# yl4579/StyleTTS2

Hardware: AMD Instinct MI355X
Metric: audio-seconds/sec (RTF^-1) end-to-end, 10 s utterance batch (higher is better)
Workload: dtype f32 (convs/linears: f16 hi/lo split, 3 MFMA products, fp32 accumulate)

## Files before the change

### styletts2_amd/_build.py

```python
import os
import subprocess
import sys

HERE = os.path.dirname(os.path.abspath(__file__))
CSRC = os.path.join(HERE, "csrc")
INCLUDE = os.path.join(os.path.dirname(HERE), "include")
LIB_PATH = os.path.join(HERE, "libst2_hip.so")

SOURCES = ["st2_api.hip", "st2_conv1d.hip", "st2_conv1d_f16s.hip", "st2_conv1d_f16s_k0.hip", "st2_conv1d_f16s_k1.hip",
           "st2_conv1d_f16s_k2.hip", "st2_conv1d_f16s_w0.hip", "st2_conv1d_f16s_w1.hip", "st2_conv1d_f16s_w2.hip",
           "st2_conv1d_xs.hip", "st2_conv1d_xs_k0.hip", "st2_conv1d_xs_k1.hip",
           "st2_conv1d_xs_k2.hip", "st2_conv1d_xs_k3.hip", "st2_actsplit.hip", "st2_norm.hip", "st2_misc.hip", "st2_glue.hip", "st2_pack.hip", "st2_resample.hip", "st2_passage.hip", "st2_level.hip", "st2_limit.hip", "st2_rng.hip", "st2_fit.hip", "st2_ingest.hip", "st2_controls.hip", "st2_marks.hip", "st2_style.hip", "st2_engine.hip", "st2_source.hip", "st2_attention.hip", "st2_lstm.hip", "st2_lstm_coop.hip", "st2_probe.hip", "st2_probe_conv.hip"]
FLAGS = ["--offload-arch=gfx950", "-O3", "-std=c++17", "-ffp-contract=off", "-fPIC", "-Wall",
         "-Wno-unused-function", "-I" + INCLUDE, "-I" + CSRC]
EXTRA_FLAGS = {s: ["-fno-slp-vectorize"] for s in SOURCES if s.startswith("st2_conv1d_f16s_k")}
EXTRA_FLAGS.update({"st2_lstm.hip": ["-fno-slp-vectorize"], "st2_lstm_coop.hip": ["-fno-slp-vectorize"]})
EXTRA_FLAGS.update({"st2_resample.hip": ["-fno-slp-vectorize"], "st2_ingest.hip": ["-fno-slp-vectorize"]})
EXTRA_FLAGS.update({"st2_level.hip": ["-fno-slp-vectorize"]})
EXTRA_FLAGS.update({"st2_limit.hip": ["-fno-slp-vectorize"]})


def _hipcc():
    for c in (os.environ.get("HIPCC"), "/opt/rocm/bin/hipcc", "hipcc"):
        if c and (os.path.isabs(c) and os.path.exists(c) or not os.path.isabs(c)):
            return c
    raise RuntimeError("hipcc not found")


def _newer(src_list, target):
    if not os.path.exists(target):
        return True
    t = os.path.getmtime(target)
    return any((not os.path.exists(s)) or os.path.getmtime(s) > t for s in src_list)


def _depfile_inputs(depfile):
    try:
        text = open(depfile).read()
    except OSError:
        return None
    text = text.replace("\\\n", " ")
    if ":" not in text:
        return None
    deps = text.split(":", 1)[1].split()
    return [d for d in deps if not d.startswith("/opt/rocm") and not d.startswith("/usr/")] or None


def _stale(src, obj, flags):
    stamp = obj + ".flags"
    try:
        if open(stamp).read() != " ".join(flags):
            return True
    except OSError:
        return True
    deps = _depfile_inputs(obj[:-2] + ".d")
    return deps is None or _newer([src] + deps, obj)


def build_lib(force=False, verbose=True):
    hipcc = _hipcc()
    objdir = os.path.join(CSRC, "build")
    os.makedirs(objdir, exist_ok=True)
    objs = []
    procs = []
    for s in SOURCES:
        src = os.path.join(CSRC, s)
        obj = os.path.join(objdir, s.replace(".hip", ".o"))
        objs.append(obj)
        flags = FLAGS + EXTRA_FLAGS.get(s, [])
        if force or _stale(src, obj, flags):
            cmd = [hipcc] + flags + ["-MD", "-MF", obj[:-2] + ".d", "-c", src, "-o", obj]
            if verbose:
                print("[st2 build]", " ".join(cmd), flush=True)
            if os.path.exists(obj + ".flags"):
                os.remove(obj + ".flags")
            procs.append((s, obj, flags, subprocess.Popen(cmd)))
    for s, obj, flags, p in procs:
        if p.wait() != 0:
            raise RuntimeError("hipcc failed on %s" % s)
        with open(obj + ".flags", "w") as f:
            f.write(" ".join(flags))
    if force or procs or _newer(objs, LIB_PATH):
        cmd = [hipcc, "--offload-arch=gfx950", "-shared", "-fPIC", "-o", LIB_PATH] + objs
        if verbose:
            print("[st2 build]", " ".join(cmd), flush=True)
        subprocess.check_call(cmd)
        isa_gate(verbose)
    return LIB_PATH


def isa_gate(verbose=True):
    import importlib.util
    path = os.path.join(os.path.dirname(HERE), "tools", "check_isa.py")
    spec = importlib.util.spec_from_file_location("st2_check_isa", path)
    mod = importlib.util.module_from_spec(spec)
    spec.loader.exec_module(mod)
    ok, report = mod.check(LIB_PATH)
    if verbose or ok is False:
        print("[st2 build] " + report, flush=True)
    if ok is False:
        os.replace(LIB_PATH, LIB_PATH + ".rejected")
        raise RuntimeError("libst2_hip.so failed the ISA gate (tools/check_isa.py); kept as %s.rejected" % LIB_PATH)
    return ok


if __name__ == "__main__":
    build_lib(force="--force" in sys.argv)
    print(LIB_PATH)
```

### styletts2_amd/csrc/st2_misc.hip

```cpp
#include "st2_common.h"

namespace {

__global__ __launch_bounds__(256) void conv1d_direct_kernel(const float* __restrict__ x, int64_t x_bs, int x_cs,
                                                            const float* __restrict__ w,
                                                            const float* __restrict__ bias, float* __restrict__ y,
                                                            int64_t y_bs, int y_cs, int C_in, int L_in_max, int L_out,
                                                            int ks, int stride, int pad, const int32_t* __restrict__ x_len,
                                                            const int32_t* __restrict__ y_len) {
  const int l = blockIdx.x * 256 + threadIdx.x;
  const int co = blockIdx.y;
  const int b = blockIdx.z;
  if (l >= L_out) return;
  const int L_in = x_len ? min(x_len[b], L_in_max) : L_in_max;
  if (y_len && l >= y_len[b]) {
    y[(int64_t)b * y_bs + (int64_t)co * y_cs + l] = 0.f;
    return;
  }
  const float* xb = x + (int64_t)b * x_bs;
  const float* wc = w + (int64_t)co * C_in * ks;
  float acc = 0.f;
  const int base = l * stride - pad;
  for (int ci = 0; ci < C_in; ++ci) {
    const float* xr = xb + (int64_t)ci * x_cs;
    for (int t = 0; t < ks; ++t) {
      const int p = base + t;
      if (p >= 0 && p < L_in) acc = fmaf(wc[ci * ks + t], xr[p], acc);
    }
  }
  if (bias) acc += bias[co];
  y[(int64_t)b * y_bs + (int64_t)co * y_cs + l] = acc;
}

__global__ __launch_bounds__(256) void phase_split_kernel(const float* __restrict__ x, int64_t x_bs, int x_cs, int L_in,
                                                          float* __restrict__ xp, int64_t p_bs, int p_cs, int Lu,
                                                          int stride, int pad) {
  const int pp = blockIdx.x * 256 + threadIdx.x;
  const int ci = blockIdx.y;
  const int b = blockIdx.z;
  if (pp >= Lu * stride) return;
  const int u = pp / stride;
  const int r = pp - u * stride;
  const int p = pp - pad;
  const float v = (p >= 0 && p < L_in) ? x[(int64_t)b * x_bs + (int64_t)ci * x_cs + p] : 0.f;
  xp[(int64_t)b * p_bs + (int64_t)(ci * stride + r) * p_cs + u] = v;
}

constexpr int CVT_TILE = 1024;
template <int S>
__global__ __launch_bounds__(256) void convt_interleave_kernel(const float* __restrict__ ph, int64_t p_bs, int p_cs,
                                                               const float* __restrict__ bias,
                                                               const float* __restrict__ add, int64_t a_bs, int a_cs,
                                                               float* __restrict__ out, int64_t o_bs, int o_cs, int C,
                                                               int stride_rt, int pad, int L_raw_max, int reflect_left,
                                                               float* __restrict__ part, int part_nt, int Lq_max,
                                                               const int32_t* __restrict__ q_len,
                                                               const int32_t* __restrict__ out_len) {
  extern __shared__ float cvt_tile[];
  __shared__ float red[2][4];
  const int stride = S ? S : stride_rt;
  const int co = blockIdx.y;
  const int b = blockIdx.z;
  const int L_out = out_len ? min(out_len[b], L_raw_max + reflect_left) : L_raw_max + reflect_left;
  const int Lq = q_len ? min(q_len[b], Lq_max) : Lq_max;
  const int o0 = blockIdx.x * CVT_TILE;
  if (o0 >= L_out) return;
  const int nq = CVT_TILE / stride + 3;
  const int nqp = nq | 1;
  const int l_lo = max(o0 - reflect_left, 0);
  const int q_lo = (l_lo + pad) / stride;
  {
    const float* pb = ph + (int64_t)b * p_bs + (int64_t)co * p_cs;
    const int total = stride * nq;
    constexpr int SB = 8;
    for (int e0 = threadIdx.x; e0 < total; e0 += 256 * SB) {
      float t[SB];
#pragma unroll
      for (int u = 0; u < SB; ++u) {
        const int e = min(e0 + u * 256, total - 1);
        const int r = e / nq, i = e - r * nq;
        t[u] = pb[(int64_t)r * C * p_cs + max(min(q_lo + i, Lq - 1), 0)];
      }
#pragma unroll
      for (int u = 0; u < SB; ++u) {
        const int e = e0 + u * 256;
        if (e < total) {
          const int r = e / nq, i = e - r * nq;
          cvt_tile[r * nqp + i] = (q_lo + i) < Lq ? t[u] : 0.f;
        }
      }
    }
  }
  __syncthreads();
  const float bj = bias ? bias[co] : 0.f;
  const float* ab = add ? add + (int64_t)b * a_bs + (int64_t)co * a_cs : nullptr;
  float* ob = out + (int64_t)b * o_bs + (int64_t)co * o_cs;
  auto staged_at = [&](int o) __attribute__((always_inline)) -> float {
    int l = o;
    if (reflect_left) l = (o == 0) ? 1 : o - 1;
    const int lp = l + pad;
    const int q = lp / stride;
    const int r = lp - q * stride;
    return cvt_tile[r * nqp + (q - q_lo)] + bj;
  };
  float shift = staged_at(o0);
  if (ab) shift += ab[o0];
  float s1 = 0.f, s2 = 0.f;
  const int o = o0 + 4 * threadIdx.x;
  if (o < L_out) {
    typedef float f4 __attribute__((ext_vector_type(4)));
    const bool full = o + 3 < L_out;
    const bool vec = full && ((reinterpret_cast<uintptr_t>(ob + o) & 15) == 0) && (!ab || (reinterpret_cast<uintptr_t>(ab + o) & 15) == 0);
    float v[4];
#pragma unroll
    for (int e = 0; e < 4; ++e) v[e] = (full || o + e < L_out) ? staged_at(o + e) : 0.f;
    if (ab) {
      if (vec) {
        const f4 a4 = *reinterpret_cast<const f4*>(ab + o);
#pragma unroll
        for (int e = 0; e < 4; ++e) v[e] += a4[e];
      } else {
#pragma unroll
        for (int e = 0; e < 4; ++e)
          if (full || o + e < L_out) v[e] += ab[o + e];
      }
    }
    if (vec) {
      *reinterpret_cast<f4*>(ob + o) = f4{v[0], v[1], v[2], v[3]};
    } else {
#pragma unroll
      for (int e = 0; e < 4; ++e)
        if (full || o + e < L_out) ob[o + e] = v[e];
    }
#pragma unroll
    for (int e = 0; e < 4; ++e)
      if (full || o + e < L_out) {
        const float dv = v[e] - shift;
        s1 += dv;
        s2 += dv * dv;
      }
  }
  if (part) {
    s1 = st2_wave_sum(s1);
    s2 = st2_wave_sum(s2);
    const int lane = threadIdx.x & 63, wave = threadIdx.x >> 6;
    if (lane == 0) {
      red[0][wave] = s1;
      red[1][wave] = s2;
    }
    __syncthreads();
    if (threadIdx.x == 0) {
      const float t1 = ((red[0][0] + red[0][1]) + red[0][2]) + red[0][3];
      const float t2 = ((red[1][0] + red[1][1]) + red[1][2]) + red[1][3];
      const int64_t slot = ((int64_t)b * C + co) * part_nt + blockIdx.x;
      reinterpret_cast<float2*>(part)[slot] = make_float2(t1, t2);
      part[(int64_t)gridDim.z * C * part_nt * 2 + slot] = shift;
    }
  }
}

__global__ __launch_bounds__(256) void adain_leaky_pool_kernel(const float* __restrict__ x, int64_t x_bs, int x_cs,
                                                               const float* __restrict__ stats,
                                                               const float* __restrict__ gamma,
                                                               const float* __restrict__ beta, int64_t gb_bs,
                                                               float slope, const float* __restrict__ w,
                                                               const float* __restrict__ bias, float* __restrict__ y,
                                                               int64_t y_bs, int y_cs, int C, int L_max,
                                                               const int32_t* __restrict__ len) {
  const int lo = blockIdx.x * 256 + threadIdx.x;
  const int c = blockIdx.y;
  const int b = blockIdx.z;
  const int L = len ? min(len[b], L_max) : L_max;
  if (lo >= 2 * L) return;
  const float mean = stats[((int64_t)b * C + c) * 2 + 0];
  const float rstd = stats[((int64_t)b * C + c) * 2 + 1];
  const float g = 1.0f + gamma[(int64_t)b * gb_bs + c];
  const float be = beta[(int64_t)b * gb_bs + c];
  const float* xr = x + (int64_t)b * x_bs + (int64_t)c * x_cs;
  auto act = [&](int i) -> float {
    float u = (xr[i] - mean) * rstd;
    u = g * u + be;
    return u >= 0.f ? u : u * slope;
  };
  const int j = lo >> 1;
  float v;
  if ((lo & 1) == 0) {
    v = act(j) * w[c * 3 + 1];
  } else {
    v = act(j) * w[c * 3 + 2];
    if (j + 1 < L) v += act(j + 1) * w[c * 3 + 0];
  }
  if (bias) v += bias[c];
  y[(int64_t)b * y_bs + (int64_t)c * y_cs + lo] = v;
}

__global__ __launch_bounds__(256) void add_chanvec_kernel(const float* __restrict__ x, int64_t x_bs, int x_cs,
                                                          const float* __restrict__ v, int64_t v_bs,
                                                          float* __restrict__ y, int64_t y_bs, int y_cs, int C,
                                                          int N) {
  const int n = blockIdx.x * 256 + threadIdx.x;
  const int c = blockIdx.y;
  const int b = blockIdx.z;
  if (n >= N) return;
  y[(int64_t)b * y_bs + (int64_t)c * y_cs + n] =
      x[(int64_t)b * x_bs + (int64_t)c * x_cs + n] + v[(int64_t)b * v_bs + c];
}

__global__ __launch_bounds__(64) void mean_tokens_kernel(const float* __restrict__ x, int64_t x_bs, int x_cs,
                                                         float* __restrict__ m, int64_t m_bs, int C, int N,
                                                         const int* __restrict__ len) {
  const int c = blockIdx.x;
  const int b = blockIdx.y;
  const float* xr = x + (int64_t)b * x_bs + (int64_t)c * x_cs;
  const int n_b = len ? min(max(len[b], 1), N) : N;
  double s = 0.0;
  for (int n = threadIdx.x; n < n_b; n += 64) s += (double)xr[n];
  s = st2_wave_sum(s);
  if (threadIdx.x == 0) m[(int64_t)b * m_bs + c] = (float)(s / (double)n_b);
}

__global__ __launch_bounds__(256) void axpbypcz_kernel(const float* __restrict__ x, float a,
                                                       const float* __restrict__ y, float b,
                                                       const float* __restrict__ z, float c, float* __restrict__ out,
                                                       int64_t n) {
  const int64_t i = (int64_t)blockIdx.x * 256 + threadIdx.x;
  if (i >= n) return;
  float v = a * x[i];
  if (y) v += b * y[i];
  if (z) v += c * z[i];
  out[i] = v;
}

}

extern "C" int st2_conv1d_direct(const float* x, int64_t x_bs, int32_t x_cs, const float* w, const float* bias,
                                 float* y, int64_t y_bs, int32_t y_cs, int32_t B, int32_t C_in, int32_t C_out,
                                 int32_t L_in, int32_t L_out, int32_t ks, int32_t stride, int32_t pad,
                                 void* stream) {
  return st2_conv1d_direct_len(x, x_bs, x_cs, w, bias, y, y_bs, y_cs, B, C_in, C_out, L_in, L_out, ks, stride, pad, nullptr,
                               nullptr, stream);
}

extern "C" int st2_conv1d_direct_len(const float* x, int64_t x_bs, int32_t x_cs, const float* w, const float* bias,
                                     float* y, int64_t y_bs, int32_t y_cs, int32_t B, int32_t C_in, int32_t C_out,
                                     int32_t L_in, int32_t L_out, int32_t ks, int32_t stride, int32_t pad,
                                     const int32_t* x_len, const int32_t* y_len, void* stream) {
  ST2_REQUIRE(x && w && y && B > 0 && C_in > 0 && C_out > 0 && L_in > 0 && L_out > 0 && ks > 0 && stride > 0,
              "st2_conv1d_direct: bad arguments");
  ST2_REQUIRE(C_out <= 65535 && B <= 65535, "st2_conv1d_direct: grid too large");
  hipStream_t s = reinterpret_cast<hipStream_t>(stream);
  hipLaunchKernelGGL(conv1d_direct_kernel, dim3(st2_cdiv(L_out, 256), C_out, B), dim3(256), 0, s, x, x_bs, x_cs, w,
                     bias, y, y_bs, y_cs, C_in, L_in, L_out, ks, stride, pad, x_len, y_len);
  ST2_CHECK_LAUNCH("st2_conv1d_direct");
  return 0;
}

extern "C" int st2_phase_split(const float* x, int64_t x_bs, int32_t x_cs, int32_t B, int32_t C, int32_t L_in,
                               int32_t stride, int32_t pad, float* xp, int64_t p_bs, int32_t p_cs, int32_t Lu,
                               void* stream) {
  ST2_REQUIRE(x && xp && B > 0 && C > 0 && L_in > 0 && stride > 0 && pad >= 0 && Lu > 0,
              "st2_phase_split: bad arguments");
  ST2_REQUIRE(C <= 65535 && B <= 65535 && (int64_t)Lu * stride < (int64_t)1 << 31, "st2_phase_split: grid too large");
  hipStream_t s = reinterpret_cast<hipStream_t>(stream);
  hipLaunchKernelGGL(phase_split_kernel, dim3(st2_cdiv((int64_t)Lu * stride, 256), C, B), dim3(256), 0, s, x, x_bs,
                     x_cs, L_in, xp, p_bs, p_cs, Lu, stride, pad);
  ST2_CHECK_LAUNCH("st2_phase_split");
  return 0;
}

extern "C" int st2_convt_interleave(const float* phases, int64_t p_bs, int32_t p_cs, int32_t Lq, const float* bias,
                                    const float* add, int64_t a_bs, int32_t a_cs, float* out, int64_t o_bs,
                                    int32_t o_cs, int32_t B, int32_t C, int32_t stride, int32_t pad, int32_t L_raw,
                                    int32_t reflect_left, void* stream) {
  return st2_convt_interleave_stats(phases, p_bs, p_cs, Lq, bias, add, a_bs, a_cs, out, o_bs, o_cs, B, C, stride, pad,
                                    L_raw, reflect_left, nullptr, 0, stream);
}

extern "C" int st2_convt_interleave_stats(const float* phases, int64_t p_bs, int32_t p_cs, int32_t Lq,
                                          const float* bias, const float* add, int64_t a_bs, int32_t a_cs, float* out,
                                          int64_t o_bs, int32_t o_cs, int32_t B, int32_t C, int32_t stride, int32_t pad,
                                          int32_t L_raw, int32_t reflect_left, float* part, int32_t part_nt,
                                          void* stream) {
  return st2_convt_interleave_stats_len(phases, p_bs, p_cs, Lq, bias, add, a_bs, a_cs, out, o_bs, o_cs, B, C, stride, pad, L_raw,
                                        reflect_left, part, part_nt, nullptr, nullptr, stream);
}

extern "C" int st2_convt_interleave_stats_len(const float* phases, int64_t p_bs, int32_t p_cs, int32_t Lq,
                                              const float* bias, const float* add, int64_t a_bs, int32_t a_cs, float* out,
                                              int64_t o_bs, int32_t o_cs, int32_t B, int32_t C, int32_t stride, int32_t pad,
                                              int32_t L_raw, int32_t reflect_left, float* part, int32_t part_nt,
                                              const int32_t* q_len, const int32_t* out_len, void* stream) {
  ST2_REQUIRE(!q_len == !out_len, "st2_convt_interleave_stats_len: q_len and out_len go together");
  ST2_REQUIRE(phases && out && B > 0 && C > 0 && stride > 0 && L_raw > 0 && Lq > 0,
              "st2_convt_interleave: bad arguments");
  ST2_REQUIRE(reflect_left == 0 || (reflect_left == 1 && L_raw >= 2), "st2_convt_interleave: bad reflect_left");
  ST2_REQUIRE(stride <= 64, "st2_convt_interleave: stride %d too large", stride);
  const int L_out = L_raw + reflect_left;
  const int nt = st2_cdiv(L_out, CVT_TILE);
  if (part) ST2_REQUIRE(part_nt >= nt && (reinterpret_cast<uintptr_t>(part) & 7) == 0,
                        "st2_convt_interleave: part_nt=%d < %d tiles (or part not 8-byte aligned)", part_nt, nt);
  ST2_REQUIRE(B <= 65535 && C <= 65535, "st2_convt_interleave: grid too large");
  hipStream_t s = reinterpret_cast<hipStream_t>(stream);
  const int nq = CVT_TILE / stride + 3;
  const size_t smem = (size_t)stride * (nq | 1) * sizeof(float);
#define ST2_CVT_LAUNCH(SV)                                                                                              \
  hipLaunchKernelGGL((convt_interleave_kernel<SV>), dim3(nt, C, B), dim3(256), smem, s, phases, p_bs, p_cs, bias, add, \
                     a_bs, a_cs, out, o_bs, o_cs, C, stride, pad, L_raw, reflect_left, part, part_nt, Lq, q_len, out_len)
  switch (stride) {
    case 2: ST2_CVT_LAUNCH(2); break;
    case 3: ST2_CVT_LAUNCH(3); break;
    case 5: ST2_CVT_LAUNCH(5); break;
    case 6: ST2_CVT_LAUNCH(6); break;
    case 10: ST2_CVT_LAUNCH(10); break;
    default: ST2_CVT_LAUNCH(0); break;
  }
#undef ST2_CVT_LAUNCH
  ST2_CHECK_LAUNCH("st2_convt_interleave");
  return 0;
}

extern "C" int st2_convt_interleave_part_cols(void) { return CVT_TILE; }

extern "C" int st2_adain_leaky_pool(const float* x, int64_t x_bs, int32_t x_cs, const float* stats,
                                    const float* gamma, const float* beta, int64_t gb_bs, float slope, const float* w,
                                    const float* bias, float* y, int64_t y_bs, int32_t y_cs, int32_t B, int32_t C,
                                    int32_t L, void* stream) {
  return st2_adain_leaky_pool_len(x, x_bs, x_cs, stats, gamma, beta, gb_bs, slope, w, bias, y, y_bs, y_cs, B, C, L, nullptr,
                                  stream);
}

extern "C" int st2_adain_leaky_pool_len(const float* x, int64_t x_bs, int32_t x_cs, const float* stats,
                                        const float* gamma, const float* beta, int64_t gb_bs, float slope, const float* w,
                                        const float* bias, float* y, int64_t y_bs, int32_t y_cs, int32_t B, int32_t C,
                                        int32_t L, const int32_t* len, void* stream) {
  ST2_REQUIRE(x && stats && gamma && beta && w && y && B > 0 && C > 0 && L > 0,
              "st2_adain_leaky_pool: bad arguments");
  hipStream_t s = reinterpret_cast<hipStream_t>(stream);
  hipLaunchKernelGGL(adain_leaky_pool_kernel, dim3(st2_cdiv(2 * L, 256), C, B), dim3(256), 0, s, x, x_bs, x_cs,
                     stats, gamma, beta, gb_bs, slope, w, bias, y, y_bs, y_cs, C, L, len);
  ST2_CHECK_LAUNCH("st2_adain_leaky_pool");
  return 0;
}

extern "C" int st2_add_chanvec(const float* x, int64_t x_bs, int32_t x_cs, const float* v, int64_t v_bs, float* y,
                               int64_t y_bs, int32_t y_cs, int32_t B, int32_t C, int32_t N, void* stream) {
  ST2_REQUIRE(x && v && y && B > 0 && C > 0 && N > 0, "st2_add_chanvec: bad arguments");
  hipStream_t s = reinterpret_cast<hipStream_t>(stream);
  hipLaunchKernelGGL(add_chanvec_kernel, dim3(st2_cdiv(N, 256), C, B), dim3(256), 0, s, x, x_bs, x_cs, v, v_bs, y,
                     y_bs, y_cs, C, N);
  ST2_CHECK_LAUNCH("st2_add_chanvec");
  return 0;
}

extern "C" int st2_mean_tokens(const float* x, int64_t x_bs, int32_t x_cs, float* m, int64_t m_bs, int32_t B,
                               int32_t C, int32_t N, void* stream) {
  ST2_REQUIRE(x && m && B > 0 && C > 0 && N > 0, "st2_mean_tokens: bad arguments");
  hipStream_t s = reinterpret_cast<hipStream_t>(stream);
  hipLaunchKernelGGL(mean_tokens_kernel, dim3(C, B), dim3(64), 0, s, x, x_bs, x_cs, m, m_bs, C, N,
                     static_cast<const int*>(nullptr));
  ST2_CHECK_LAUNCH("st2_mean_tokens");
  return 0;
}

extern "C" int st2_mean_tokens_len(const float* x, int64_t x_bs, int32_t x_cs, float* m, int64_t m_bs, int32_t B,
                                   int32_t C, int32_t N, const int32_t* len, void* stream) {
  ST2_REQUIRE(x && m && B > 0 && C > 0 && N > 0, "st2_mean_tokens_len: bad arguments");
  hipStream_t s = reinterpret_cast<hipStream_t>(stream);
  hipLaunchKernelGGL(mean_tokens_kernel, dim3(C, B), dim3(64), 0, s, x, x_bs, x_cs, m, m_bs, C, N,
                     reinterpret_cast<const int*>(len));
  ST2_CHECK_LAUNCH("st2_mean_tokens_len");
  return 0;
}

extern "C" int st2_axpbypcz(const float* x, float a, const float* y, float b, const float* z, float c, float* out,
                            int64_t n, void* stream) {
  ST2_REQUIRE(x && out && n > 0, "st2_axpbypcz: bad arguments");
  hipStream_t s = reinterpret_cast<hipStream_t>(stream);
  hipLaunchKernelGGL(axpbypcz_kernel, dim3(st2_cdiv(n, 256)), dim3(256), 0, s, x, a, y, b, z, c, out, n);
  ST2_CHECK_LAUNCH("st2_axpbypcz");
  return 0;
}
```

### styletts2_amd/csrc/st2_source.hip

```cpp
#include "st2_common.h"

namespace {

__device__ __forceinline__ float torch_remainder1(float x) {
  float m = fmodf(x, 1.0f);
  if (m != 0.0f && m < 0.0f) m += 1.0f;
  return m;
}

__global__ __launch_bounds__(64) void sinegen_phase_kernel(const float* __restrict__ f0, int B, int F_max, int U, int H,
                                                           float sample_rate, float* __restrict__ phase_f,
                                                           const int32_t* __restrict__ f_len) {
  const int row = blockIdx.x;
  const int lane = threadIdx.x;
  const int b = row / H;
  const int h = row % H;
  const float mult = (float)(h + 1);
  const int F = f_len ? min(f_len[b], F_max) : F_max;
  const float* f = f0 + (int64_t)b * F_max;
  float* out = phase_f + ((int64_t)b * H + h) * F_max;
  const float two_pi_part = 3.14159274101257324219f;
  const float fu = (float)U;
  const int chunk = (F + 63) / 64;
  const int k0 = min(lane * chunk, F), k1 = min(k0 + chunk, F);
  double part = 0.0;
  for (int k = k0; k < k1; ++k) {
    const float fn = f[k] * mult;
    part += (double)torch_remainder1(fn / sample_rate);
  }
  double incl = part;
#pragma unroll
  for (int d = 1; d < 64; d <<= 1) {
    const double up = __shfl_up(incl, d, 64);
    if (lane >= d) incl += up;
  }
  double acc = __shfl_up(incl, 1, 64);
  if (lane == 0) acc = 0.0;
  for (int k = k0; k < k1; ++k) {
    const float fn = f[k] * mult;
    acc += (double)torch_remainder1(fn / sample_rate);
    const float c = (float)acc;
    out[k] = ((c * 2.0f) * two_pi_part) * fu;
  }
}

__global__ __launch_bounds__(256) void har_source_kernel(const float* __restrict__ f0, int F_max, int U, int H,
                                                         const float* __restrict__ noise,
                                                         const float* __restrict__ lin_w,
                                                         const float* __restrict__ lin_b, float sine_amp,
                                                         float noise_std, float voiced_threshold,
                                                         const float* __restrict__ phase_f,
                                                         float* __restrict__ out, const int32_t* __restrict__ f_len) {
  const int L_max = F_max * U;
  const int t = blockIdx.x * 256 + threadIdx.x;
  const int b = blockIdx.y;
  if (t >= L_max) return;
  const int F = f_len ? min(f_len[b], F_max) : F_max;
  const int L = F * U;
  if (t >= L) {
    out[(int64_t)b * L_max + t] = 0.f;
    return;
  }
  const float rs = (float)(1.0 / (double)U);
  float src = fmaf(rs, (float)t + 0.5f, -0.5f);
  src = src < 0.f ? 0.f : src;
  const int i0 = (int)src;
  const int i1 = min(i0 + 1, F - 1);
  const float w1 = src - (float)i0;
  const float w0 = 1.0f - w1;

  const float f0v = f0[(int64_t)b * F_max + t / U];
  const float uv = f0v > voiced_threshold ? 1.0f : 0.0f;
  const float noise_amp = uv * noise_std + ((1.0f - uv) * sine_amp) / 3.0f;

  const float* nz = noise + ((int64_t)b * L_max + t) * H;
  float acc = 0.f;
  for (int h = 0; h < H; ++h) {
    const float* pf = phase_f + ((int64_t)b * H + h) * F_max;
    const float ph = fmaf(w0, pf[i0], w1 * pf[i1]);
    const float sine = sinf(ph) * sine_amp;
    const float sw = sine * uv + noise_amp * nz[h];
    acc = fmaf(lin_w[h], sw, acc);
  }
  out[(int64_t)b * L_max + t] = tanhf(acc + lin_b[0]);
}

constexpr int MAXN = 32;
__global__ __launch_bounds__(256) void stft_kernel(const float* __restrict__ x, int L_max, int N, int hop,
                                                   float* __restrict__ har, int64_t har_bs, int har_cs,
                                                   const int32_t* __restrict__ len) {
  __shared__ float tw_c[MAXN], tw_s[MAXN], win[MAXN];
  if (threadIdx.x < N) {
    const double a = 2.0 * (double)threadIdx.x / (double)N;
    tw_c[threadIdx.x] = (float)cospi(a);
    tw_s[threadIdx.x] = (float)sinpi(a);
    win[threadIdx.x] = (float)(0.5 - 0.5 * cospi(a));
  }
  __syncthreads();
  const int m = blockIdx.x * 256 + threadIdx.x;
  const int b = blockIdx.y;
  if (m >= L_max / hop + 1) return;
  const int L = len ? min(max(len[b], N / 2 + 1), L_max) : L_max;
  const int M = L / hop + 1;
  const int NB = N / 2 + 1;
  float* hb = har + (int64_t)b * har_bs + m;
  if (m >= M) {
    for (int k = 0; k < 2 * NB; ++k) hb[(int64_t)k * har_cs] = 0.f;
    return;
  }
  const float* xb = x + (int64_t)b * L_max;
  float fr[MAXN];
  const int pad = N / 2;
#pragma unroll
  for (int n = 0; n < MAXN; ++n) {
    if (n < N) {
      int i = m * hop + n - pad;
      if (i < 0) i = -i;
      if (i >= L) i = 2 * (L - 1) - i;
      fr[n] = xb[i] * win[n];
    } else {
      fr[n] = 0.f;
    }
  }
  for (int k = 0; k < NB; ++k) {
    float re = 0.f, im = 0.f;
    int idx = 0;
#pragma unroll
    for (int n = 0; n < MAXN; ++n) {
      if (n < N) {
        re = fmaf(fr[n], tw_c[idx], re);
        im = fmaf(-fr[n], tw_s[idx], im);
        idx += k;
        if (idx >= N) idx -= N;
      }
    }
    hb[(int64_t)k * har_cs] = sqrtf(re * re + im * im);
    hb[(int64_t)(NB + k) * har_cs] = atan2f(im, re);
  }
}

__global__ __launch_bounds__(256) void istft_kernel(const float* __restrict__ sp, int64_t sp_bs, int sp_cs, int M_max,
                                                    int N, int hop, float* __restrict__ wave, int64_t wave_bs, int FRP,
                                                    const int32_t* __restrict__ m_len) {
  __shared__ float tw_c[MAXN], tw_s[MAXN], win[MAXN];
  extern __shared__ float ri[];
  if (threadIdx.x < N) {
    const double a = 2.0 * (double)threadIdx.x / (double)N;
    tw_c[threadIdx.x] = (float)cospi(a);
    tw_s[threadIdx.x] = (float)sinpi(a);
    win[threadIdx.x] = (float)(0.5 - 0.5 * cospi(a));
  }
  const int t = blockIdx.x * 256 + threadIdx.x;
  const int b = blockIdx.y;
  const int M = m_len ? min(max(m_len[b], 2), M_max) : M_max;
  const int Lw = hop * (M - 1);
  const int NB = N / 2 + 1;
  const float* sb = sp + (int64_t)b * sp_bs;
  {
    const int t0 = blockIdx.x * 256;
    const int tp0 = t0 + N / 2, tp1 = min(t0 + 255, Lw - 1) + N / 2;
    const int m_base = (tp0 - N + 1 <= 0) ? 0 : (tp0 - N + hop) / hop;
    const int m_last = min(tp1 / hop, M - 1);
    const int FR = m_last - m_base + 1;
    float* re_s = ri;
    float* im_s = ri + NB * FRP;
    for (int e = threadIdx.x; e < NB * FR; e += 256) {
      const int k = e / FR, f = e - k * FR;
      const float mag = sb[(int64_t)k * sp_cs + m_base + f];
      const float ph = sb[(int64_t)(NB + k) * sp_cs + m_base + f];
      re_s[k * FRP + f] = mag * cosf(ph);
      im_s[k * FRP + f] = mag * sinf(ph);
    }
  }
  __syncthreads();
  if (t >= Lw) {
    if (t < hop * (M_max - 1)) wave[(int64_t)b * wave_bs + t] = 0.f;
    return;
  }
  const int tp = t + N / 2;
  const int tp0 = (int)blockIdx.x * 256 + N / 2;
  const int m_base = (tp0 - N + 1 <= 0) ? 0 : (tp0 - N + hop) / hop;
  const float* re_s = ri;
  const float* im_s = ri + NB * FRP;
  int m_hi = tp / hop;
  if (m_hi > M - 1) m_hi = M - 1;
  int m_lo = (tp - N + hop) / hop;
  if (tp - N + 1 <= 0) m_lo = 0;
  const float inv_n = 1.0f / (float)N;
  float y = 0.f, env = 0.f;
  for (int m = m_lo; m <= m_hi; ++m) {
    const int n = tp - m * hop;
    float acc = 0.f;
    int idx = 0;
    const int f = m - m_base;
    for (int k = 0; k < NB; ++k) {
      const float re = re_s[k * FRP + f];
      const float im = im_s[k * FRP + f];
      if (k == 0 || k == N / 2) {
        acc += re * tw_c[idx];
      } else {
        acc += 2.0f * (re * tw_c[idx] - im * tw_s[idx]);
      }
      idx += n;
      if (idx >= N) idx -= N;
    }
    const float w = win[n];
    y += (acc * inv_n) * w;
    env += w * w;
  }
  wave[(int64_t)b * wave_bs + t] = y / env;
}

}

extern "C" int st2_har_source(const float* f0, int32_t B, int32_t F, int32_t U, int32_t H, const float* noise,
                              const float* lin_w, const float* lin_b, float sine_amp, float noise_std,
                              float voiced_threshold, float sample_rate, float* phase_scratch, float* out,
                              void* stream) {
  return st2_har_source_len(f0, B, F, U, H, noise, lin_w, lin_b, sine_amp, noise_std, voiced_threshold, sample_rate,
                            phase_scratch, out, nullptr, stream);
}

extern "C" int st2_har_source_len(const float* f0, int32_t B, int32_t F, int32_t U, int32_t H, const float* noise,
                                  const float* lin_w, const float* lin_b, float sine_amp, float noise_std,
                                  float voiced_threshold, float sample_rate, float* phase_scratch, float* out,
                                  const int32_t* f_len, void* stream) {
  ST2_REQUIRE(f0 && noise && lin_w && lin_b && phase_scratch && out, "st2_har_source: null pointer");
  ST2_REQUIRE(B > 0 && F > 0 && U > 0 && H > 0 && H <= 64, "st2_har_source: bad geometry");
  ST2_REQUIRE((int64_t)F * U < (1LL << 31), "st2_har_source: utterance too long");
  hipStream_t s = reinterpret_cast<hipStream_t>(stream);
  hipLaunchKernelGGL(sinegen_phase_kernel, dim3(B * H), dim3(64), 0, s, f0, B, F, U, H, sample_rate,
                     phase_scratch, f_len);
  ST2_CHECK_LAUNCH("st2_har_source(phase)");
  hipLaunchKernelGGL(har_source_kernel, dim3(st2_cdiv((int64_t)F * U, 256), B), dim3(256), 0, s, f0, F, U, H, noise,
                     lin_w, lin_b, sine_amp, noise_std, voiced_threshold, phase_scratch, out, f_len);
  ST2_CHECK_LAUNCH("st2_har_source");
  return 0;
}

extern "C" int st2_stft_mag_phase(const float* x, int32_t B, int32_t L, int32_t n_fft, int32_t hop, float* har,
                                  int64_t har_bs, int32_t har_cs, void* stream) {
  return st2_stft_mag_phase_len(x, B, L, n_fft, hop, har, har_bs, har_cs, nullptr, stream);
}

extern "C" int st2_stft_mag_phase_len(const float* x, int32_t B, int32_t L, int32_t n_fft, int32_t hop, float* har,
                                      int64_t har_bs, int32_t har_cs, const int32_t* len, void* stream) {
  ST2_REQUIRE(x && har && B > 0 && L > 0, "st2_stft_mag_phase: bad arguments");
  ST2_REQUIRE(n_fft >= 2 && n_fft <= MAXN && (n_fft % 2) == 0 && hop > 0 && L > n_fft / 2,
              "st2_stft_mag_phase: n_fft=%d hop=%d L=%d unsupported", n_fft, hop, L);
  hipStream_t s = reinterpret_cast<hipStream_t>(stream);
  const int M = L / hop + 1;
  hipLaunchKernelGGL(stft_kernel, dim3(st2_cdiv(M, 256), B), dim3(256), 0, s, x, L, n_fft, hop, har, har_bs, har_cs, len);
  ST2_CHECK_LAUNCH("st2_stft_mag_phase");
  return 0;
}

extern "C" int st2_istft(const float* sp, int64_t sp_bs, int32_t sp_cs, int32_t B, int32_t M, int32_t n_fft,
                         int32_t hop, float* wave, int64_t wave_bs, void* stream) {
  return st2_istft_len(sp, sp_bs, sp_cs, B, M, n_fft, hop, wave, wave_bs, nullptr, stream);
}

extern "C" int st2_istft_len(const float* sp, int64_t sp_bs, int32_t sp_cs, int32_t B, int32_t M, int32_t n_fft,
                             int32_t hop, float* wave, int64_t wave_bs, const int32_t* m_len, void* stream) {
  ST2_REQUIRE(sp && wave && B > 0 && M > 1, "st2_istft: bad arguments");
  ST2_REQUIRE(n_fft >= 2 && n_fft <= MAXN && (n_fft % 2) == 0 && hop > 0 && (n_fft % hop) == 0,
              "st2_istft: n_fft=%d hop=%d unsupported", n_fft, hop);
  hipStream_t s = reinterpret_cast<hipStream_t>(stream);
  const int Lw = hop * (M - 1);
  const int FRP = (256 / hop + n_fft / hop + 3) | 1;
  const size_t smem = (size_t)2 * (n_fft / 2 + 1) * FRP * sizeof(float);
  hipLaunchKernelGGL(istft_kernel, dim3(st2_cdiv(Lw, 256), B), dim3(256), smem, s, sp, sp_bs, sp_cs, M, n_fft, hop, wave,
                     wave_bs, FRP, m_len);
  ST2_CHECK_LAUNCH("st2_istft");
  return 0;
}
```

Baseline: 5108.

## Batch loads in small kernels: direct conv, convtranspose epilogue, pool, harmonic source

Several small kernels get their memory access reworked. The direct conv1d loads weights and inputs in unrolled chunks of 16 with clamped indices and predicated FMAs. The transposed-conv epilogue prefetches the residual add with nontemporal loads before the barrier. The adain-leaky-pool kernel computes four outputs per thread with vector loads and stores. The harmonic source kernel stages its noise tile in shared memory through coalesced nontemporal loads instead of strided per-thread reads. These changes target memory latency and uncoalesced access in minor kernels, at the cost of more registers and shared memory.

Result: no change. 5119, median of 6 (+0.2%).

```diff
diff --git a/styletts2_amd/_build.py b/styletts2_amd/_build.py
--- a/styletts2_amd/_build.py
+++ b/styletts2_amd/_build.py
@@ -18,6 +18,7 @@
 EXTRA_FLAGS.update({"st2_resample.hip": ["-fno-slp-vectorize"], "st2_ingest.hip": ["-fno-slp-vectorize"]})
 EXTRA_FLAGS.update({"st2_level.hip": ["-fno-slp-vectorize"]})
 EXTRA_FLAGS.update({"st2_limit.hip": ["-fno-slp-vectorize"]})
+EXTRA_FLAGS.update({"st2_misc.hip": ["-fno-slp-vectorize"]})
 
 
 def _hipcc():
diff --git a/styletts2_amd/csrc/st2_misc.hip b/styletts2_amd/csrc/st2_misc.hip
--- a/styletts2_amd/csrc/st2_misc.hip
+++ b/styletts2_amd/csrc/st2_misc.hip
@@ -21,12 +21,25 @@
   const float* wc = w + (int64_t)co * C_in * ks;
   float acc = 0.f;
   const int base = l * stride - pad;
-  for (int ci = 0; ci < C_in; ++ci) {
-    const float* xr = xb + (int64_t)ci * x_cs;
-    for (int t = 0; t < ks; ++t) {
+  constexpr int DCH = 16;
+  const int total = C_in * ks;
+  int ci = 0, t = 0;
+  for (int e0 = 0; e0 < total; e0 += DCH) {
+    float xv[DCH], wv[DCH];
+    bool ok[DCH];
+#pragma unroll
+    for (int u = 0; u < DCH; ++u) {
       const int p = base + t;
-      if (p >= 0 && p < L_in) acc = fmaf(wc[ci * ks + t], xr[p], acc);
-    }
+      ok[u] = e0 + u < total && p >= 0 && p < L_in;
+      xv[u] = xb[(int64_t)min(ci, C_in - 1) * x_cs + max(min(p, L_in - 1), 0)];
+      wv[u] = wc[min(e0 + u, total - 1)];
+      if (++t == ks) {
+        t = 0;
+        ++ci;
+      }
+    }
+#pragma unroll
+    for (int u = 0; u < DCH; ++u) acc = ok[u] ? fmaf(wv[u], xv[u], acc) : acc;
   }
   if (bias) acc += bias[co];
   y[(int64_t)b * y_bs + (int64_t)co * y_cs + l] = acc;
@@ -79,7 +92,7 @@
       for (int u = 0; u < SB; ++u) {
         const int e = min(e0 + u * 256, total - 1);
         const int r = e / nq, i = e - r * nq;
-        t[u] = pb[(int64_t)r * C * p_cs + max(min(q_lo + i, Lq - 1), 0)];
+        t[u] = __builtin_nontemporal_load(&pb[(int64_t)r * C * p_cs + max(min(q_lo + i, Lq - 1), 0)]);
       }
 #pragma unroll
       for (int u = 0; u < SB; ++u) {
@@ -91,10 +104,28 @@
       }
     }
   }
-  __syncthreads();
   const float bj = bias ? bias[co] : 0.f;
   const float* ab = add ? add + (int64_t)b * a_bs + (int64_t)co * a_cs : nullptr;
   float* ob = out + (int64_t)b * o_bs + (int64_t)co * o_cs;
+  typedef float f4 __attribute__((ext_vector_type(4)));
+  const int o = o0 + 4 * threadIdx.x;
+  const bool full = o + 3 < L_out;
+  const bool vec = full && ((reinterpret_cast<uintptr_t>(ob + o) & 15) == 0) && (!ab || (reinterpret_cast<uintptr_t>(ab + o) & 15) == 0);
+  float av[4] = {0.f, 0.f, 0.f, 0.f};
+  float a_first = 0.f;
+  if (ab) {
+    a_first = ab[o0];
+    if (vec) {
+      const f4 a4 = __builtin_nontemporal_load(reinterpret_cast<const f4*>(ab + o));
+#pragma unroll
+      for (int e = 0; e < 4; ++e) av[e] = a4[e];
+    } else {
+#pragma unroll
+      for (int e = 0; e < 4; ++e)
+        if (o + e < L_out) av[e] = __builtin_nontemporal_load(ab + o + e);
+    }
+  }
+  __syncthreads();
   auto staged_at = [&](int o) __attribute__((always_inline)) -> float {
     int l = o;
     if (reflect_left) l = (o == 0) ? 1 : o - 1;
@@ -104,26 +135,16 @@
     return cvt_tile[r * nqp + (q - q_lo)] + bj;
   };
   float shift = staged_at(o0);
-  if (ab) shift += ab[o0];
+  if (ab) shift += a_first;
   float s1 = 0.f, s2 = 0.f;
-  const int o = o0 + 4 * threadIdx.x;
   if (o < L_out) {
-    typedef float f4 __attribute__((ext_vector_type(4)));
-    const bool full = o + 3 < L_out;
-    const bool vec = full && ((reinterpret_cast<uintptr_t>(ob + o) & 15) == 0) && (!ab || (reinterpret_cast<uintptr_t>(ab + o) & 15) == 0);
     float v[4];
 #pragma unroll
     for (int e = 0; e < 4; ++e) v[e] = (full || o + e < L_out) ? staged_at(o + e) : 0.f;
     if (ab) {
-      if (vec) {
-        const f4 a4 = *reinterpret_cast<const f4*>(ab + o);
-#pragma unroll
-        for (int e = 0; e < 4; ++e) v[e] += a4[e];
-      } else {
-#pragma unroll
-        for (int e = 0; e < 4; ++e)
-          if (full || o + e < L_out) v[e] += ab[o + e];
-      }
+#pragma unroll
+      for (int e = 0; e < 4; ++e)
+        if (full || o + e < L_out) v[e] += av[e];
     }
     if (vec) {
       *reinterpret_cast<f4*>(ob + o) = f4{v[0], v[1], v[2], v[3]};
@@ -167,31 +188,58 @@
                                                                const float* __restrict__ bias, float* __restrict__ y,
                                                                int64_t y_bs, int y_cs, int C, int L_max,
                                                                const int32_t* __restrict__ len) {
-  const int lo = blockIdx.x * 256 + threadIdx.x;
+  const int j0 = (blockIdx.x * 256 + threadIdx.x) * 2;
   const int c = blockIdx.y;
   const int b = blockIdx.z;
   const int L = len ? min(len[b], L_max) : L_max;
-  if (lo >= 2 * L) return;
+  if (j0 >= L) return;
   const float mean = stats[((int64_t)b * C + c) * 2 + 0];
   const float rstd = stats[((int64_t)b * C + c) * 2 + 1];
   const float g = 1.0f + gamma[(int64_t)b * gb_bs + c];
   const float be = beta[(int64_t)b * gb_bs + c];
   const float* xr = x + (int64_t)b * x_bs + (int64_t)c * x_cs;
-  auto act = [&](int i) -> float {
-    float u = (xr[i] - mean) * rstd;
+  auto act = [&](float xv) -> float {
+    float u = (xv - mean) * rstd;
     u = g * u + be;
     return u >= 0.f ? u : u * slope;
   };
-  const int j = lo >> 1;
-  float v;
-  if ((lo & 1) == 0) {
-    v = act(j) * w[c * 3 + 1];
+  const bool has1 = j0 + 1 < L, has2 = j0 + 2 < L;
+  float x0, x1 = 0.f;
+  if (has1 && (reinterpret_cast<uintptr_t>(xr + j0) & 7) == 0) {
+    const float2 x01 = *reinterpret_cast<const float2*>(xr + j0);
+    x0 = x01.x;
+    x1 = x01.y;
   } else {
-    v = act(j) * w[c * 3 + 2];
-    if (j + 1 < L) v += act(j + 1) * w[c * 3 + 0];
-  }
-  if (bias) v += bias[c];
-  y[(int64_t)b * y_bs + (int64_t)c * y_cs + lo] = v;
+    x0 = xr[j0];
+    if (has1) x1 = xr[j0 + 1];
+  }
+  const float x2 = has2 ? xr[j0 + 2] : 0.f;
+  const float a0 = act(x0), a1 = act(x1), a2 = act(x2);
+  const float w0 = w[c * 3 + 0], w1 = w[c * 3 + 1], w2 = w[c * 3 + 2];
+  float v[4];
+  v[0] = a0 * w1;
+  v[1] = a0 * w2;
+  if (has1) v[1] += a1 * w0;
+  v[2] = a1 * w1;
+  v[3] = a1 * w2;
+  if (has2) v[3] += a2 * w0;
+  if (bias) {
+    const float bc = bias[c];
+#pragma unroll
+    for (int e = 0; e < 4; ++e) v[e] += bc;
+  }
+  float* yr = y + (int64_t)b * y_bs + (int64_t)c * y_cs + 2 * j0;
+  if (has1 && (reinterpret_cast<uintptr_t>(yr) & 15) == 0) {
+    typedef float f4 __attribute__((ext_vector_type(4)));
+    *reinterpret_cast<f4*>(yr) = f4{v[0], v[1], v[2], v[3]};
+  } else {
+    yr[0] = v[0];
+    yr[1] = v[1];
+    if (has1) {
+      yr[2] = v[2];
+      yr[3] = v[3];
+    }
+  }
 }
 
 __global__ __launch_bounds__(256) void add_chanvec_kernel(const float* __restrict__ x, int64_t x_bs, int x_cs,
@@ -336,7 +384,7 @@
   ST2_REQUIRE(x && stats && gamma && beta && w && y && B > 0 && C > 0 && L > 0,
               "st2_adain_leaky_pool: bad arguments");
   hipStream_t s = reinterpret_cast<hipStream_t>(stream);
-  hipLaunchKernelGGL(adain_leaky_pool_kernel, dim3(st2_cdiv(2 * L, 256), C, B), dim3(256), 0, s, x, x_bs, x_cs,
+  hipLaunchKernelGGL(adain_leaky_pool_kernel, dim3(st2_cdiv(L, 512), C, B), dim3(256), 0, s, x, x_bs, x_cs,
                      stats, gamma, beta, gb_bs, slope, w, bias, y, y_bs, y_cs, C, L, len);
   ST2_CHECK_LAUNCH("st2_adain_leaky_pool");
   return 0;
diff --git a/styletts2_amd/csrc/st2_source.hip b/styletts2_amd/csrc/st2_source.hip
--- a/styletts2_amd/csrc/st2_source.hip
+++ b/styletts2_amd/csrc/st2_source.hip
@@ -50,13 +50,30 @@
                                                          const float* __restrict__ lin_b, float sine_amp,
                                                          float noise_std, float voiced_threshold,
                                                          const float* __restrict__ phase_f,
-                                                         float* __restrict__ out, const int32_t* __restrict__ f_len) {
+                                                         float* __restrict__ out, const int32_t* __restrict__ f_len,
+                                                         int staged) {
+  extern __shared__ float nz_s[];
   const int L_max = F_max * U;
-  const int t = blockIdx.x * 256 + threadIdx.x;
+  const int t0 = blockIdx.x * 256;
+  const int t = t0 + threadIdx.x;
   const int b = blockIdx.y;
-  if (t >= L_max) return;
   const int F = f_len ? min(f_len[b], F_max) : F_max;
   const int L = F * U;
+  if (staged && t0 < L) {
+    const int n = min(256, L_max - t0) * H;
+    const float* src = noise + ((int64_t)b * L_max + t0) * H;
+    if ((reinterpret_cast<uintptr_t>(src) & 15) == 0) {
+      typedef float f4 __attribute__((ext_vector_type(4)));
+      const int n4 = n >> 2;
+      for (int i = threadIdx.x; i < n4; i += 256)
+        *reinterpret_cast<f4*>(nz_s + 4 * i) = __builtin_nontemporal_load(reinterpret_cast<const f4*>(src) + i);
+      for (int i = 4 * n4 + threadIdx.x; i < n; i += 256) nz_s[i] = __builtin_nontemporal_load(src + i);
+    } else {
+      for (int i = threadIdx.x; i < n; i += 256) nz_s[i] = __builtin_nontemporal_load(src + i);
+    }
+  }
+  __syncthreads();
+  if (t >= L_max) return;
   if (t >= L) {
     out[(int64_t)b * L_max + t] = 0.f;
     return;
@@ -73,7 +90,7 @@
   const float uv = f0v > voiced_threshold ? 1.0f : 0.0f;
   const float noise_amp = uv * noise_std + ((1.0f - uv) * sine_amp) / 3.0f;
 
-  const float* nz = noise + ((int64_t)b * L_max + t) * H;
+  const float* nz = staged ? nz_s + threadIdx.x * H : noise + ((int64_t)b * L_max + t) * H;
   float acc = 0.f;
   for (int h = 0; h < H; ++h) {
     const float* pf = phase_f + ((int64_t)b * H + h) * F_max;
@@ -232,8 +249,10 @@
   hipLaunchKernelGGL(sinegen_phase_kernel, dim3(B * H), dim3(64), 0, s, f0, B, F, U, H, sample_rate,
                      phase_scratch, f_len);
   ST2_CHECK_LAUNCH("st2_har_source(phase)");
-  hipLaunchKernelGGL(har_source_kernel, dim3(st2_cdiv((int64_t)F * U, 256), B), dim3(256), 0, s, f0, F, U, H, noise,
-                     lin_w, lin_b, sine_amp, noise_std, voiced_threshold, phase_scratch, out, f_len);
+  const int staged = H <= 32;
+  hipLaunchKernelGGL(har_source_kernel, dim3(st2_cdiv((int64_t)F * U, 256), B), dim3(256),
+                     staged ? (size_t)256 * H * sizeof(float) : 0, s, f0, F, U, H, noise, lin_w, lin_b, sine_amp, noise_std,
+                     voiced_threshold, phase_scratch, out, f_len, staged);
   ST2_CHECK_LAUNCH("st2_har_source");
   return 0;
 }
```
